# TSultanov/cfd-demo

Hardware: AMD Instinct MI355X
Metric: cell-updates/s (Poisson iter) + ms/timestep, 4096² grid, 1/2/4/8 GPU (higher is better)
Workload: dtype f32

## Files before the change

### cfd-demo_amd/cfdamd/__init__.py

```python
from __future__ import annotations

import ctypes as C
import enum
from dataclasses import dataclass
from typing import List, Optional, Tuple

import numpy as np

from . import _lib
from ._lib import (CFD_ENONFINITE, CfdError, CfdGrid, CfdParams, CfdResiduals, CfdState, check,
                   load)

__all__ = [
    "VelocityScheme", "InletProfile", "PressureSolver", "BoundaryKind", "Cylinder", "Grid",
    "SimulationParams", "Residuals", "SimSnapshot", "Model", "SimulationControlHandle",
    "CfdError", "default_grid", "cavity_grid", "rccl_unique_id", "device_count", "load", "LocalHub",
    "VisualizationMode", "CFD_ENONFINITE", "ScriptScheme", "ScriptPhase", "ScriptReport",
]


class VelocityScheme(enum.IntEnum):
    FirstOrder = 0
    SecondOrder = 1

# ... 464 lines not shown
        mm = np.empty(2, np.float32)
        check("cfd_derive_field", load().cfd_derive_field(self._hh(), int(mode), _fp(out), _fp(mm)))
        return out, (float(mm[0]), float(mm[1]))

    def launches_per_solve(self) -> int:
        tmax = self.kernel_config["temporal"]
        iters = self.params.jacobi_iters
        hg = self.halo_depth if self.n_ranks > 1 else 0
        T, lo, hi, ex = C.c_int(), C.c_int(), C.c_int(), C.c_int()
        it = n = 0
        while it < iters:
            check("cfd_plan_block", load().cfd_plan_block(
                self.j0, self.nyl, self.grid.ny, hg, it, tmax, iters, C.byref(T), C.byref(lo),
                C.byref(hi), C.byref(ex)))
            it += T.value
            n += 1
        return n

    @property
    def jacobi_kernel(self) -> dict:
        kind, name = C.c_int(), C.create_string_buffer(96)
        check("cfd_get_jacobi_kernel",
              load().cfd_get_jacobi_kernel(self._hh(), C.byref(kind), name, 96))
        return {"kind": kind.value, "name": name.value.decode()}

    def jacobi_geometry(self, persist: bool = True) -> dict:
        v = [C.c_int32() for _ in range(4)]
        check("cfd_get_jacobi_geometry",
              load().cfd_get_jacobi_geometry(self._hh(), int(bool(persist)), *(C.byref(x) for x in v)))
        return dict(lds_pad=v[0].value, wgs_per_cu=v[1].value, wave_cols=v[2].value,
                    segments=v[3].value)

    @property
    def persist_steals(self) -> int:
        n = C.c_uint64()
        check("cfd_get_persist_steals", load().cfd_get_persist_steals(self._hh(), C.byref(n)))
        return int(n.value)

    @property
    def persist_sums(self) -> int:
        n = C.c_uint64()
        check("cfd_get_persist_sums", load().cfd_get_persist_sums(self._hh(), C.byref(n)))
        return int(n.value)

    @property
    def sums_launches(self) -> int:
        n = C.c_uint64()
        check("cfd_get_sums_launches", load().cfd_get_sums_launches(self._hh(), C.byref(n)))
        return int(n.value)

    @property
    def sums_bounds(self) -> dict:
        s, a, b = C.c_uint32(), C.c_uint32(), C.c_uint32()
        check("cfd_get_sums_bounds",
              load().cfd_get_sums_bounds(self._hh(), C.byref(s), C.byref(a), C.byref(b)))
        return {"state": int(s.value), "m0": int(a.value), "rm": int(b.value)}

    @property
    def comm_calls(self) -> int:
        n = C.c_uint64()
        check("cfd_get_comm_calls", load().cfd_get_comm_calls(self._hh(), C.byref(n)))
        return int(n.value)

    @property
    def recoveries(self) -> int:
        n = C.c_uint64()
# ... 192 lines not shown
```

### cfd-demo_amd/cfdamd/_lib.py

```python
from __future__ import annotations

import ctypes as C
import os

PKG_DIR = os.path.dirname(os.path.abspath(__file__))
ROOT = os.path.dirname(PKG_DIR)
LIB_PATH = os.environ.get("CFD_LIB") or os.path.join(ROOT, "lib", "libcfd_amd.so")

EXPORTS = [
    "cfd_default_params", "cfd_default_grid", "cfd_create", "cfd_rccl_unique_id",
    "cfd_create_sharded", "cfd_local_hub_create", "cfd_local_hub_destroy",
    "cfd_create_sharded_local", "cfd_device_count", "cfd_get_comm_size", "cfd_get_slab", "cfd_update", "cfd_update_n", "cfd_piso_step",
    "cfd_pressure_solve", "cfd_run_phase", "cfd_set_params", "cfd_get_snapshot",
    "cfd_get_residuals", "cfd_get_state", "cfd_set_state", "cfd_get_masks", "cfd_synchronize",
    "cfd_profile_sweeps", "cfd_timing_begin", "cfd_timing_end", "cfd_timing_phases",
    "cfd_timing_phase_ms", "cfd_timing_exchange_ms", "cfd_get_halo_depth",
    "cfd_get_kernel_config", "cfd_get_jacobi_kernel", "cfd_get_persist_blocks", "cfd_get_persist_steals", "cfd_get_persist_sums", "cfd_get_sums_launches", "cfd_get_sums_bounds", "cfd_get_recoveries", "cfd_get_comm_calls", "cfd_get_resident_solves", "cfd_get_resident_geometry", "cfd_get_jacobi_geometry", "cfd_plan_slab", "cfd_plan_sweep", "cfd_plan_halo", "cfd_plan_block", "cfd_plan_overlap",
    "cfd_render", "cfd_derive_field", "cfd_last_error", "cfd_abi_version", "cfd_destroy",
    "cfd_get_config", "cfd_run_start", "cfd_run_stop", "cfd_run_pause", "cfd_run_resume",
    "cfd_run_set_params", "cfd_run_request_snapshot", "cfd_run_last_snapshot",
    "cfd_run_new_residuals", "cfd_run_status", "cfd_run_steps",
    "cfd_polygon_new", "cfd_polygon_new_rect", "cfd_polygon_new_regular", "cfd_polygon_add_hole",
    "cfd_polygon_contains_point", "cfd_polygon_intersects_aabb",
    "cfd_polygon_edges_intersect_aabb", "cfd_polygon_bounding_box",
    "cfd_polygon_bounding_square", "cfd_polygon_edges", "cfd_polygon_destroy",
    "cfd_geom_do_intersect", "cfd_geom_segment_intersection", "cfd_geom_intersect_quad_edge",
    "cfd_tesselate", "cfd_quadtree_size", "cfd_quadtree_nodes", "cfd_quadtree_destroy",
    "cfd_mesh_from_quadtree", "cfd_mesh_sizes", "cfd_mesh_cells", "cfd_mesh_neighbors",
    "cfd_mesh_intersections", "cfd_mesh_full_bounding_box", "cfd_mesh_build_ms",
    "cfd_mesh_destroy",
    "cfd_tracers_enable", "cfd_tracers_disable", "cfd_tracers_count", "cfd_tracers_get",
    "cfd_tracers_set", "cfd_tracers_advance", "cfd_tracers_inject", "cfd_tracers_density",
    "cfd_run_set_tracers", "cfd_run_last_tracers",
    "cfd_script_piso_step", "cfd_script_phase",
    "cfd_script_begin", "cfd_script_get_state", "cfd_script_set_state", "cfd_script_update",
    "cfd_script_update_n",
    "cfd_script_set_options", "cfd_script_get_options", "cfd_get_p_residual_f64",
]


class CfdGrid(C.Structure):
    _fields_ = [("nx", C.c_uint64), ("ny", C.c_uint64), ("lx", C.c_float), ("ly", C.c_float),
                ("has_cylinder", C.c_int32), ("cylinder_x", C.c_float),
                ("cylinder_y", C.c_float), ("cylinder_radius", C.c_float)]


class CfdParams(C.Structure):
    _fields_ = [("dt", C.c_float), ("viscosity", C.c_float),
                ("target_inlet_velocity", C.c_float), ("velocity_scheme", C.c_int32),
                ("inlet_profile", C.c_int32), ("pressure_solver", C.c_int32),
# ... 94 lines not shown
        "cfd_update_n": (i32, [vp, i32]),
        "cfd_piso_step": (i32, [vp, f32]),
        "cfd_pressure_solve": (i32, [vp, FP]),
        "cfd_run_phase": (i32, [vp, i32, f32]),
        "cfd_set_params": (i32, [vp, C.POINTER(CfdParams)]),
        "cfd_get_snapshot": (i32, [vp, FP, FP, FP, FP]),
        "cfd_get_residuals": (i32, [vp, C.POINTER(CfdResiduals)]),
        "cfd_get_state": (i32, [vp, C.POINTER(CfdState)]),
        "cfd_set_state": (i32, [vp, C.POINTER(CfdState)]),
        "cfd_get_masks": (i32, [vp, C.POINTER(C.c_uint8), C.POINTER(C.c_uint8)]),
        "cfd_synchronize": (i32, [vp]),
        "cfd_profile_sweeps": (i32, [vp, i32, C.POINTER(C.c_double)]),
        "cfd_timing_begin": (i32, [vp]),
        "cfd_timing_end": (i32, [vp, C.POINTER(C.c_double), C.POINTER(C.c_uint64),
                                 C.POINTER(C.c_double), C.POINTER(C.c_uint64)]),
        "cfd_timing_phases": (i32, [vp, i32]),
        "cfd_timing_phase_ms": (i32, [vp, C.POINTER(C.c_double), C.POINTER(C.c_double)]),
        "cfd_timing_exchange_ms": (i32, [vp, C.POINTER(C.c_double), C.POINTER(C.c_uint64)]),
        "cfd_get_halo_depth": (i32, [vp]),
        "cfd_get_kernel_config": (i32, [vp, C.POINTER(i32), C.POINTER(i32)]),
        "cfd_get_jacobi_kernel": (i32, [vp, C.POINTER(i32), C.c_char_p, C.c_size_t]),
        "cfd_get_persist_blocks": (i32, [vp, C.POINTER(i32)]),
        "cfd_get_persist_steals": (i32, [vp, C.POINTER(C.c_uint64)]),
        "cfd_get_persist_sums": (i32, [vp, C.POINTER(C.c_uint64)]),
        "cfd_get_sums_launches": (i32, [vp, C.POINTER(C.c_uint64)]),
        "cfd_get_sums_bounds": (i32, [vp, C.POINTER(C.c_uint32), C.POINTER(C.c_uint32),
                                      C.POINTER(C.c_uint32)]),
        "cfd_get_recoveries": (i32, [vp, C.POINTER(C.c_uint64)]),
        "cfd_get_comm_calls": (i32, [vp, C.POINTER(C.c_uint64)]),
        "cfd_get_resident_solves": (i32, [vp, C.POINTER(C.c_uint64)]),
        "cfd_get_resident_geometry": (i32, [vp] + [C.POINTER(i32)] * 4),
        "cfd_get_jacobi_geometry": (i32, [vp, i32, C.POINTER(i32), C.POINTER(i32), C.POINTER(i32),
                                          C.POINTER(i32)]),
        "cfd_plan_slab": (i32, [C.c_uint64, i32, i32, C.POINTER(C.c_uint64),
                                C.POINTER(C.c_uint64)]),
        "cfd_plan_sweep": (i32, [i32, i32, i32, i32, i32, i32, C.POINTER(i32), C.POINTER(i32),
                                 C.POINTER(i32)]),
        "cfd_plan_halo": (i32, [i32, i32, i32, i32, i32, C.POINTER(i32)]),
        "cfd_plan_overlap": (i32, [i32, i32, i32, i32, i32, i32, C.POINTER(i32)]),
        "cfd_plan_block": (i32, [i32, i32, i32, i32, i32, i32, i32, C.POINTER(i32),
                                 C.POINTER(i32), C.POINTER(i32), C.POINTER(i32)]),
        "cfd_render": (i32, [vp, i32, C.POINTER(C.c_uint8), FP]),
        "cfd_derive_field": (i32, [vp, i32, FP, FP]),
        "cfd_last_error": (C.c_char_p, []),
        "cfd_abi_version": (i32, []),
        "cfd_destroy": (None, [vp]),
        "cfd_get_config": (i32, [vp, C.POINTER(CfdGrid), C.POINTER(CfdParams)]),
        "cfd_run_start": (i32, [vp, C.POINTER(vp)]),
        "cfd_run_stop": (i32, [vp]),
        "cfd_run_pause": (i32, [vp]),
        "cfd_run_resume": (i32, [vp]),
        "cfd_run_set_params": (i32, [vp, C.POINTER(CfdParams)]),
        "cfd_run_request_snapshot": (i32, [vp]),
        "cfd_run_last_snapshot": (i32, [vp, FP, FP, FP, FP, C.POINTER(i32), C.POINTER(i32)]),
        "cfd_run_new_residuals": (i32, [vp, C.POINTER(CfdResiduals), i32, C.POINTER(i32)]),
        "cfd_run_status": (i32, [vp, C.c_char_p, C.c_size_t]),
        "cfd_run_steps": (C.c_uint64, [vp]),
        "cfd_polygon_new": (i32, [C.POINTER(CfdPoint), C.c_size_t, C.POINTER(C.c_uint64),
                                  C.c_size_t, C.POINTER(vp), C.POINTER(i32)]),
        "cfd_polygon_new_rect": (i32, [C.c_double] * 4 + [C.POINTER(vp)]),
        "cfd_polygon_new_regular": (i32, [CfdPoint, C.c_double, C.c_size_t, C.c_double,
                                          C.POINTER(vp)]),
        "cfd_polygon_add_hole": (i32, [vp, vp, C.POINTER(i32)]),
        "cfd_polygon_contains_point": (i32, [vp, CfdPoint, C.POINTER(i32)]),
        "cfd_polygon_intersects_aabb": (i32, [vp, C.POINTER(CfdAabb), C.POINTER(i32)]),
        "cfd_polygon_edges_intersect_aabb": (i32, [vp, C.POINTER(CfdAabb), C.POINTER(i32)]),
# ... 59 lines not shown
```

### cfd-demo_amd/csrc/cfd_internal.h

```cpp
#pragma once
#include <hip/hip_runtime.h>
#include <stdint.h>

#include <type_traits>

#include "../../include/cfd.h"

namespace cfd {

template <class Fn>
auto with_fastdiv(int fastdiv, Fn &&f) {
    if (fastdiv == 1) return f(std::integral_constant<int, 1>{});
    if (fastdiv == 2) return f(std::integral_constant<int, 2>{});
    return f(std::integral_constant<int, 0>{});
}

constexpr int kGhostUV = 2;
constexpr float kSumsPLim = 0x1p122f, kSumsRLim = 0x1p112f;
constexpr int kMaxSweeps = 4096;
constexpr int kMaxPasses = 64;

constexpr int kResSlots = 32;
constexpr int kResStride = 16;
constexpr int kPersistFlagStride = 16;
// ... 68 lines not shown
    size_t u_alloc, v_alloc;
    float *u_alloc_base, *v_alloc_base, *u_old_base, *v_old_base, *u_star_base, *v_star_base;
    Ctl *ctl;
    uint32_t *host_nonfinite;
    uint32_t *host_progress;
    uint32_t *persist;
    int32_t sums_track;
};

inline bool aligned16(const void *p) { return ((uintptr_t)p & 15u) == 0; }

void launch_step_begin(const Geom &g, const Fields &f, int copy, hipStream_t s);
void launch_copy_star(const Geom &g, const Fields &f, int pass, hipStream_t s);
void launch_copy_star_div(const Geom &g, const Fields &f, int pass, float dt_override,
                          hipStream_t s);
void launch_u_predictor(const Geom &g, const Fields &f, float dt_override, hipStream_t s);
void launch_v_predictor(const Geom &g, const Fields &f, float dt_override, hipStream_t s);
void launch_predict(const Geom &g, const Fields &f, float dt_override, bool vec, hipStream_t s);
bool predict_march_ok(const Geom &g, const Fields &f);
int predict_march_workgroups(const Geom &g);
void launch_predict_march(const Geom &g, const Fields &f, float dt_override, hipStream_t s,
                          bool set_inlet = false, int row_lo = 0, int row_hi = -1, int mode = 0,
                          bool star = false);
void launch_divergence(const Geom &g, const Fields &f, int pass, float dt_override,
                       hipStream_t s);
void launch_jacobi_sweep(const Geom &g, const Fields &f, int pass, int it, int row_lo,
                         int row_hi, int res, hipStream_t s);
void launch_jacobi_block(const Geom &g, const Fields &f, int pass, int it, int par, int T,
                         int out_lo, int out_hi, int res, hipStream_t s);
bool launch_jacobi_persist(const Geom &g, const Fields &f, int pass, int par0, int nblk,
                           int out_lo, int out_hi, uint32_t epoch, int res_it, hipStream_t s);
void lds_geometry8(const Geom &g, int out_lo, int out_hi, bool persist, int *pad, int *occ, int *nwc,
                   int *nseg);
void launch_tb1(const Geom &g, const Fields &f, int T, int pass, int it, int par, int out_lo,
                int out_hi, uint32_t *res_slots, hipStream_t s);
void launch_pipe(const Geom &g, const Fields &f, int T, int pass, int it, int par, int out_lo,
                 int out_hi, uint32_t *res_slots, hipStream_t s);
bool launch_lds_persist8(const Geom &g, const Fields &f, int pass, int par0, int nblk, int out_lo,
                         int out_hi, uint32_t epoch, uint32_t *rs, hipStream_t s);
void launch_lds(const Geom &g, const Fields &f, int T, int pass, int it, int par, int out_lo,
                int out_hi, uint32_t *res_slots, hipStream_t s, int mode = 0, int lag = 0);
void launch_jacobi_spec(const Geom &g, const Fields &f, int pass, int it, int par, int T,
                        int out_lo, int out_hi, hipStream_t s, int lag = 0);
void launch_spec_check(const Geom &g, const Fields &f, int pass, int it, int T, int par,
                       hipStream_t s);
bool launch_jacobi_resident(const Geom &g, const Fields &f, int pass, int iters, int fin,
                            int check_break, hipStream_t s);
bool jacobi_resident_geometry(const Geom &g, int *br, int *bc, int *tiles, int *wgs);
void launch_spec_align(const Geom &g, const Fields &f, int pass, int n, hipStream_t s);
void launch_jacobi_redo(const Geom &g, const Fields &f, int pass, int out_lo, int out_hi,
                        hipStream_t s, int last_it = 0, int last_par = 0, int last_T = 0);
void launch_fold_slots(uint32_t *dst, uint32_t *slots, int n, hipStream_t s);
void launch_vis_field(const Geom &g, const Fields &f, int mode, float *out, uint32_t *slots,
                      hipStream_t s);
void launch_vis_color(const Geom &g, const Fields &f, int mode, const float *field, uint32_t *px,
                      const uint32_t *keys, int has_cyl, float cx, float cy, float radius,
                      hipStream_t s);
void launch_verify_division(float c, float r, unsigned long long *dev_counts, hipStream_t s);
void launch_finalize_solve(const Geom &g, const Fields &f, int pass, int iters, int check_break,
                           int flips, hipStream_t s, int exact_flips = 0);

struct SorConst {
    double dx2, dy2, denom;
    double r_dx2, r_dy2, r_denom;
    int32_t fast;
};
// ... 108 lines not shown
```

### cfd-demo_amd/csrc/cfd_jacobi_lds.h

```cpp
#pragma once
#include <cmath>
#include <type_traits>

#include "cfd_device.h"

#ifndef CFD_LDS_PD
#define CFD_LDS_PD 3
#endif
#ifndef CFD_LDS_SPLIT
#define CFD_LDS_SPLIT 1
#endif
#ifndef CFD_LDS_PRIO
#define CFD_LDS_PRIO 1
#endif
#ifndef CFD_LDS_ST_AUX
#define CFD_LDS_ST_AUX 16
#endif
#ifndef CFD_LDS_SPEC_WPE
#define CFD_LDS_SPEC_WPE 5
#endif
#ifndef CFD_PERSIST_WPE
#define CFD_PERSIST_WPE 3
#endif
#ifndef CFD_LDS_STAMP
#define CFD_LDS_STAMP 0
#endif

namespace cfd {

constexpr int kLdsWaves = 4;

#if CFD_LDS_STAMP
namespace {
constexpr int kStampWaves = 1 << 15;
__device__ unsigned long long g_lds_stamp[kStampWaves * 4];
template <bool RES>
struct StampOnExit {
    unsigned long long rt0, t0;
    unsigned long long bid;
    __device__ explicit StampOnExit(int b)
        : rt0(__builtin_amdgcn_s_memrealtime()), t0(__builtin_amdgcn_s_memtime()),
          bid((unsigned long long)b) {}
    __device__ ~StampOnExit() {
        if (RES) return;
        const unsigned long long rt1 = __builtin_amdgcn_s_memrealtime();
        const unsigned long long t1 = __builtin_amdgcn_s_memtime();
        const unsigned hw = __builtin_amdgcn_s_getreg(4 | (31 << 11));
        const unsigned xcc = __builtin_amdgcn_s_getreg(20 | (31 << 11));
        const int idx = (int)blockIdx.x * kLdsWaves + ((int)threadIdx.x >> 6);
        if ((threadIdx.x & 63) == 0 && idx < kStampWaves) {
            g_lds_stamp[idx * 4 + 0] = rt0;
            g_lds_stamp[idx * 4 + 1] = rt1;
            g_lds_stamp[idx * 4 + 2] = (bid << 40) | ((t1 - t0) & 0xFFFFFFFFFFull);
            g_lds_stamp[idx * 4 + 3] = ((unsigned long long)xcc << 32) | hw;
        }
    }
};
}
extern "C" int cfd_diag_lds_stamps(unsigned long long *host, int nwaves) {
    if (nwaves > kStampWaves) nwaves = kStampWaves;
    return hipMemcpyFromSymbol(host, HIP_SYMBOL(g_lds_stamp), (size_t)nwaves * 32, 0,
                               hipMemcpyDeviceToHost) == hipSuccess ? nwaves : -1;
}
#endif

constexpr int lds_outl(int T) { return 64 - 2 * ((T + 1) / 2); }

struct LdsTiles {
    int pad, nwc, nseg, wlo, whi;
};
LdsTiles lds_tiles(const Geom &g, int T, int out_lo, int out_hi, int mode, int bpc, bool one_round);
int lds_pad_bytes(const Geom &g, int mode);
bool lds_sums_grid(const Geom &g);

void launch_lds_t567(const Geom &g, const Fields &f, int T, int pass, int par, int it, int out_lo,
                     int out_hi, uint32_t *rs, int mode, hipStream_t s, int lag);
void launch_lds_t8(const Geom &g, const Fields &f, int pass, int par, int it, int out_lo, int out_hi,
                   uint32_t *rs, int mode, hipStream_t s, int lag);
int persist_blocks_per_cu8(const Geom &g, int pad);

namespace {

typedef unsigned int u32x2 __attribute__((ext_vector_type(2)));
constexpr int lds_gcd(int a, int b) { return b == 0 ? a : lds_gcd(b, a % b); }
constexpr int lds_off(int s, int T, int G) { return s <= 0 ? 0 : ((s - 1) * G) / T; }
constexpr int lds_nw(int G) { return G > 1 ? 4 : 3; }
constexpr int ring_depth(int T, int PD, int G) {
    const int nw = lds_nw(G);
    const int q = nw / lds_gcd(nw, PD) * PD;
    const int need = T + lds_off(T, T, G) + 1;
    return ((need + q - 1) / q) * q;
}

template <int T, int FAST, int MODE, int SUMS = 0>
struct LdsMarch {
    static constexpr bool RES = MODE == 1 || MODE == 5, SPEC = MODE == 2, REDO = MODE == 3;
    static constexpr bool PERSIST = MODE == 4 || MODE == 5;
    static constexpr bool TRACK_IN = PERSIST && !SUMS;
    static constexpr bool TRACK_OUT = PERSIST;
    static_assert(!SUMS || FAST == 1, "SUMS: reciprocal multiply");
    static constexpr int PLD_AUX = PERSIST ? 16 : 0;
    static constexpr int PST_AUX = PERSIST ? 16 : CFD_LDS_ST_AUX;
    static constexpr int G = CFD_LDS_SPLIT;
    static constexpr int NW = lds_nw(G);
    static constexpr int PD = CFD_LDS_PD;
    static constexpr int OFFT = lds_off(T, T, G);
    static constexpr int D = ring_depth(T, PD, G);
    static constexpr int U = D;
    static constexpr int WARM = 2 * T + OFFT;
    static constexpr int H = (T + 1) / 2;
    static constexpr int OUTL = lds_outl(T);
    static constexpr int off(int s) { return lds_off(s, T, G); }
    static constexpr int start(int s) { return 2 * s + off(s); }
    static_assert(D % PD == 0 && D % NW == 0 && D >= T + OFFT + 1, "ring geometry");
    static_assert(G >= 1 && G <= T, "stage groups");

    f2 W[T][NW];
    f2 PQ[PD];
    f2 RQ[PD];
    f2 *ring;
    int lane;
    int k_first, S, lo_clamp, hi_clamp, nch, g_first, g_last, g_top, g_zero, row_bytes;
    int wbase;
    int ch, vo_ld, vo_st, abase, dir;
    bool e0, e1;
    float dx_sq, r_dx_sq, dy_sq, r_dy_sq, denom, r_denom;
    __amdgpu_buffer_rsrc_t rs_p, rs_r, rs_d;
    float m;
    float omax, imax, rmax;
    float mm[SPEC ? T : 1];
    int r0v, r1v;
    int nst;
    int nyl_;

    LdsMarch() = default;

    __device__ __forceinline__ int act(int vrow) const { return abase + dir * vrow; }

    template <int AUX = 0>
    __device__ __forceinline__ f2 ld(__amdgpu_buffer_rsrc_t rs, int vrow) const {
        vrow = vrow < k_first + S ? vrow : k_first + S - 1;
        int row = act(vrow);
        row = row < lo_clamp ? lo_clamp : (row > hi_clamp ? hi_clamp : row);
        const u32x2 v = __builtin_amdgcn_raw_buffer_load_b64(rs, vo_ld, (row - wbase) * row_bytes, AUX);
        return (f2){__uint_as_float(v.x), __uint_as_float(v.y)};
    }
    __device__ __forceinline__ void st(const f2 &x, int row) const {
        const u32x2 v = {__float_as_uint(x.x), __float_as_uint(x.y)};
// ... 79 lines not shown
                    }
                }
            }
            if (REDO && s == nst) {
                if (r >= r0v && r < r1v) {
                    const int ra = act(r);
                    st(n, ra);
                    if ((E & kRow) && r == g_first) st(n, g_zero);
                    if ((E & kRow) && r == g_last) st(n, g_top);
                }
            } else if (s < T) {
                if ((E & kRow) && r == g_top) n = W[s][(V_ - 1 + kW) % NW];
                W[s][V_ % NW] = n;
                if ((E & kRow) && r == g_first) W[s][(V_ - 1 + kW) % NW] = n;
            } else {
                const int ra = act(r);
                if (RES && ra >= 0 && ra < nyl_) {
                    const f2 d = n - C;
                    if (!(E & kCol)) {
                        m = fmaxf(fmaxf(m, fabsf(d.x)), fabsf(d.y));
                    } else {
                        if (e0) m = fmaxf(m, fabsf(d.x));
                        if (e1) m = fmaxf(m, fabsf(d.y));
                    }
                }
                st(n, ra);
                if ((E & kRow) && r == g_first) st(n, g_zero);
                if ((E & kRow) && r == g_last) st(n, g_top);
                if constexpr (TRACK_OUT) omax = fmaxf(fmaxf(omax, fabsf(n.x)), fabsf(n.y));
            }
        }
    }

    template <int V_, int E>
    __device__ __forceinline__ void warmup() {
        if constexpr (V_ < WARM) {
            slot<V_, 0, E>(V_);
            warmup<V_ + 1, E>();
        }
    }

    template <int J, int GUARD, int E>
    __device__ __forceinline__ void group(int base) {
        if constexpr (J < U) {
            slot<WARM + J, GUARD, E>(base + J);
            group<J + 1, GUARD, E>(base);
        }
    }

    __device__ __forceinline__ void set_prio(int done) const {
        if (!CFD_LDS_PRIO) return;
        const int rows = S - WARM, d4 = 4 * done;
        if (d4 >= 3 * rows)
            __builtin_amdgcn_s_setprio(0);
        else if (d4 >= 2 * rows)
            __builtin_amdgcn_s_setprio(1);
        else if (d4 >= rows)
            __builtin_amdgcn_s_setprio(2);
        else
            __builtin_amdgcn_s_setprio(3);
    }

    template <int E>
    __device__ __forceinline__ void run() {
        set_prio(0);
        warmup<0, E>();
        int base = WARM;
        const int full_end = WARM + ((S - WARM) / U) * U;
        for (; base < full_end; base += U) {
            set_prio(base - WARM);
            group<0, 1, E>(base);
        }
        set_prio(base - WARM);
        if (base < S) group<0, 2, E>(base);
    }
};

template <int T, int FAST, int MODE, int SUMS = 0>
__device__ __forceinline__ void lds_block(const Geom &g, float *__restrict__ pa,
                                          float *__restrict__ pb, const float *__restrict__ rhs,
                                          Ctl *ctl, uint32_t *res_slots, int par, int out_lo,
                                          int out_hi, int nwc, int nseg, int wlo, int whi, f2 *lds,
                                          int nst, int bid, float *trk = nullptr) {
    using M = LdsMarch<T, FAST, MODE, SUMS>;
    constexpr bool RES = M::RES;
    M w;
    w.nst = nst;
    const int wave = __builtin_amdgcn_readfirstlane((int)threadIdx.x >> 6);
    const int lane = (int)threadIdx.x & 63;
    if (M::PERSIST && trk && lane == 0) trk[3 * wave] = trk[3 * wave + 1] = trk[3 * wave + 2] = 0.0f;
    const int wc = bid % nwc;
    const int seg = (bid / nwc) * kLdsWaves + wave;
    const int nrows = out_hi - out_lo;
    if (seg >= nseg) return;
    const long total = nseg == 1 ? 16 : wlo + whi + 16L * (nseg - 2);
    auto cum = [&](int i) -> long { return i <= 0 ? 0 : (i >= nseg ? total : wlo + 16L * (i - 1)); };
    const int r0 = out_lo + (int)(cum(seg) * nrows / total);
    const int r1 = out_lo + (int)(cum(seg + 1) * nrows / total);
    if (r0 >= r1) return;
    const int nx = g.nx;
    w.ring = lds + wave * M::D * 64;
    w.lane = lane;
    w.nch = nx / 2;
    w.nyl_ = g.nyl;
    w.lo_clamp = -g.hg;
    w.hi_clamp = g.nyl + g.hg - 1;
    w.ch = wc * M::OUTL - M::H + lane;
    const bool in_dom = w.ch >= 0 && w.ch < w.nch;
    const bool out_lane = in_dom && lane >= M::H && lane < 64 - M::H;
    const int col = 2 * w.ch;
    w.row_bytes = nx * 4;
    constexpr int kFar = 0x7FFF0000;
    w.vo_ld = in_dom ? col * 4 : kFar;
    w.vo_st = out_lane ? col * 4 : kFar;
    const int si = (ctl->cur + par) & 1;
    float *src_alloc = si ? pb : pa;
    float *dst_alloc = si ? pa : pb;
// ... 121 lines not shown
            if (stop_s) return;
            if (spec_lag_first(g, ctl, res_slots - (size_t)lag * kResSlots * kResStride, it - lag, lag,
                               par - 1) < lag)
                return;
        } else if (ctl->spec_stop) {
            return;
        }
    }
    if constexpr (M::REDO) {
        if (lag > 0 && !ctl->spec_stop) {
            const int j = spec_lag_first(g, ctl, res_slots, it, lag, par, false);
            nst = j + 1 < lag ? j + 1 : 0;
        } else {
            nst = ctl->spec_redo;
            par = ctl->spec_launch;
        }
        if (nst <= 0) return;
    }
    if constexpr (FAST == 1 && MODE <= 1) {
        if (sums_c > 0.0f && ctl->sums_state == 2u) {
            const float bound = __uint_as_float(ctl->sums_m0) * g.r_dx_sq + sums_c * __uint_as_float(ctl->sums_rm);
            if (bound < 0x1p123f) {
                if (blockIdx.x == 0 && threadIdx.x == 0) atomicAdd(&ctl->sums_launches, 1u);
                lds_block<T, FAST, MODE, 2>(g, pa, pb, rhs, ctl, res_slots, par, out_lo, out_hi, nwc, nseg,
                                            wlo, whi, lds, nst, xcd_block(g));
                return;
            }
        }
    }
    lds_block<T, FAST, MODE>(g, pa, pb, rhs, ctl, res_slots, par, out_lo, out_hi, nwc, nseg, wlo,
                             whi, lds, nst, xcd_block(g));
}

template <int T, int FAST, int MODE>
int lds_blocks_per_cu(int pad) {
    static int cache[2] = {0, 0};
    int &nb = cache[pad > 0 ? 1 : 0];
    if (nb == 0) {
        int n = 0;
        if (hipOccupancyMaxActiveBlocksPerMultiprocessor(
                &n, reinterpret_cast<const void *>(&k_jacobi_lds<T, FAST, MODE>), kLdsWaves * 64, pad) !=
                hipSuccess ||
            n < 1)
            n = 1;
        nb = n;
    }
    return nb;
}

template <int T, int MODE>
void launch_lds_t(const Geom &g, const Fields &f, int pass, int par, int it, int out_lo, int out_hi,
                  uint32_t *rs, hipStream_t s, int lag = 0) {
    const int bpc = with_fastdiv(g.fastdiv, [&](auto F) {
        return lds_blocks_per_cu<T, F(), MODE>(lds_pad_bytes(g, MODE));
    });
    const LdsTiles t = lds_tiles(g, T, out_lo, out_hi, MODE, bpc, false);
    const dim3 grid(t.nwc * cdiv(t.nseg, kLdsWaves)), block(kLdsWaves * 64);
    float *pa = f.pp[0] - (long)g.hg * g.nx, *pb = f.pp[1] - (long)g.hg * g.nx;
    const float sums_c =
        MODE <= 1 && g.j0 == 0 && g.nyl == g.ny && lds_sums_grid(g) ? 0.1875f * kMaxSweeps : 0.0f;
    with_fastdiv(g.fastdiv, [&](auto F) {
        hipLaunchKernelGGL((k_jacobi_lds<T, F(), MODE>), grid, block, t.pad, s, g, pa, pb, f.rhs, f.ctl,
                           rs, pass, par, out_lo, out_hi, t.nwc, t.nseg, t.wlo, t.whi, it, lag, sums_c);
    });
}

template <int T>
void launch_lds_T(const Geom &g, const Fields &f, int pass, int par, int it, int out_lo, int out_hi,
                  uint32_t *rs, int mode, hipStream_t s, int lag = 0) {
    if (mode == 2) {
        launch_lds_t<T, 2>(g, f, pass, par, it, out_lo, out_hi, rs, s, lag);
        return;
    }
    if constexpr (T == 8) {
        if (mode == 3) {
            launch_lds_t<8, 3>(g, f, pass, par, it, out_lo, out_hi, rs, s, lag);
            return;
        }
    }
    if (rs)
        launch_lds_t<T, 1>(g, f, pass, par, it, out_lo, out_hi, rs, s);
    else
        launch_lds_t<T, 0>(g, f, pass, par, it, out_lo, out_hi, rs, s);
}

}
}
```

### cfd-demo_amd/csrc/cfd_jacobi_lds8.hip

```cpp
#include "cfd_jacobi_lds.h"

namespace cfd {

void launch_lds_t8(const Geom &g, const Fields &f, int pass, int par, int it, int out_lo, int out_hi,
                   uint32_t *rs, int mode, hipStream_t s, int lag) {
    launch_lds_T<8>(g, f, pass, par, it, out_lo, out_hi, rs, mode, s, lag);
}

void lds_geometry8(const Geom &g, int out_lo, int out_hi, bool persist, int *pad, int *occ, int *nwc,
                   int *nseg) {
    const int pd = lds_pad_bytes(g, 0);
    const int o = persist ? persist_blocks_per_cu8(g, pd)
                          : with_fastdiv(g.fastdiv, [&](auto F) { return lds_blocks_per_cu<8, F(), 0>(pd); });
    const LdsTiles t = lds_tiles(g, 8, out_lo, out_hi, 0, o, persist);
    if (pad) *pad = t.pad;
    if (occ) *occ = o;
    if (nwc) *nwc = t.nwc;
    if (nseg) *nseg = t.nseg;
}

}
```

### cfd-demo_amd/csrc/cfd_model_abi.hip

```cpp
#include <cstddef>
#include <cstdio>
#include <cstring>

#include "cfd_model.h"

using namespace cfd;

namespace {
thread_local std::string g_last_error;
}

int cfd::fail(int code, const std::string &msg) {
    g_last_error = msg;
    return code;
}

extern "C" {

const char *cfd_last_error(void) { return g_last_error.c_str(); }
void cfdrt_set_error(const char *msg) { g_last_error = msg ? msg : ""; }
int cfdrt_check_params(const cfd_model *m, const cfd_params *p) {
    if (!m) return fail(CFD_EINVAL, "null model");
    int rc = validate(&m->grid, p);
    if (rc) return rc;
// ... 545 lines not shown
            snprintf(buf, sizeof buf, "k_jacobi_resident<%d>", m->g.res_div);
        else if (spec)
            snprintf(buf, sizeof buf, "k_jacobi_lds<%d, %d, 2>", T, m->g.fastdiv);
        else if (k == 0)
            snprintf(buf, sizeof buf, "k_jacobi<%d, %d>", kJacRowsPerWave, m->g.fastdiv);
        else if (k == 1)
            snprintf(buf, sizeof buf, "k_jacobi_tb<%d, %d>", T, m->g.fastdiv);
        else if (k == 5)
            snprintf(buf, sizeof buf, "k_jacobi_lds<%d, %d, 0>", T, m->g.fastdiv);
        else
            snprintf(buf, sizeof buf, "k_jacobi_pipe<%d, %d>", T, m->g.fastdiv);
        snprintf(name, name_len, "%s", buf);
    }
    return 0;
}

int cfd_get_jacobi_geometry(const cfd_model *m, int persist, int *lds_pad, int *wgs_per_cu,
                            int *wave_cols, int *segments) {
    if (!m) return fail(CFD_EINVAL, "null model");
    if (hipSetDevice(m->device) != hipSuccess) return fail(CFD_EHIP, "hipSetDevice");
    int T, lo, hi, exch;
    plan_block((int)m->j0, m->g.nyl, m->g.ny, m->sharded() ? m->g.hg : 0, 0, 8,
               std::max(8, m->params.jacobi_iters), &T, &lo, &hi, &exch);
    if (!m->sharded()) lo = 1 - (int)m->j0, hi = (int)m->g.ny - 1 - (int)m->j0;
    int pad = 0, occ = 0, nwc = 0, nseg = 0;
    lds_geometry8(m->g, lo, hi, persist != 0, &pad, &occ, &nwc, &nseg);
    if (lds_pad) *lds_pad = pad;
    if (wgs_per_cu) *wgs_per_cu = occ;
    if (wave_cols) *wave_cols = nwc;
    if (segments) *segments = nseg;
    return 0;
}

int cfd_get_persist_steals(cfd_model *m, uint64_t *steals) {
    if (!m || !steals) return fail(CFD_EINVAL, "null argument");
    int rc = m->sync();
    if (rc) return rc;
    uint32_t v = 0;
    HIP_TRY(hipMemcpy(&v, m->f.persist + 2, 4, hipMemcpyDeviceToHost));
    *steals = v;
    return 0;
}

int cfd_get_persist_sums(cfd_model *m, uint64_t *blocks) {
    if (!m || !blocks) return fail(CFD_EINVAL, "null argument");
    int rc = m->sync();
    if (rc) return rc;
    uint32_t v = 0;
    HIP_TRY(hipMemcpy(&v, m->f.persist + 3, 4, hipMemcpyDeviceToHost));
    *blocks = v;
    return 0;
}

int cfd_get_sums_launches(cfd_model *m, uint64_t *launches) {
    if (!m || !launches) return fail(CFD_EINVAL, "null argument");
    Ctl c;
    int rc = m->read_ctl(&c);
    if (rc) return rc;
    *launches = c.sums_launches;
    return 0;
}

int cfd_get_sums_bounds(cfd_model *m, uint32_t *state, uint32_t *m0_bits, uint32_t *rm_bits) {
    if (!m || !state || !m0_bits || !rm_bits) return fail(CFD_EINVAL, "null argument");
    Ctl c;
    int rc = m->read_ctl(&c);
// ... 85 lines not shown
```

### include/cfd.h

```cpp
#ifndef CFD_H
#define CFD_H

#include <stddef.h>
#include <stdint.h>

#ifdef __cplusplus
extern "C" {
#endif

#define CFD_ABI_VERSION 1

typedef enum {
    CFD_OK = 0,
    CFD_EINVAL = -1,
    CFD_EHIP = -2,
    CFD_ERCCL = -3,
    CFD_ESTATE = -4,
    CFD_ENONFINITE = -5,
    CFD_ETIMEOUT = -6,
} cfd_status;

typedef struct cfd_model cfd_model;

typedef struct {
// ... 73 lines not shown
int cfd_run_phase(cfd_model *m, int phase, float dt_sub);

int cfd_set_params(cfd_model *m, const cfd_params *params);
int cfd_get_snapshot(cfd_model *m, float *u, float *v, float *p, float *dt_out);
int cfd_get_residuals(cfd_model *m, cfd_residuals *out);
int cfd_get_state(cfd_model *m, cfd_state *st);
int cfd_set_state(cfd_model *m, const cfd_state *st);
int cfd_get_masks(cfd_model *m, uint8_t *mask_u, uint8_t *mask_v);

int cfd_synchronize(cfd_model *m);
int cfd_profile_sweeps(cfd_model *m, int n_sweeps, double *avg_ms_out);

int cfd_timing_begin(cfd_model *m);
int cfd_timing_end(cfd_model *m, double *solve_ms, uint64_t *sweeps, double *step_ms,
                   uint64_t *steps);
int cfd_timing_phases(cfd_model *m, int on);
int cfd_timing_phase_ms(const cfd_model *m, double *predict_ms, double *finish_ms);
int cfd_timing_exchange_ms(const cfd_model *m, double *exchange_ms, uint64_t *exchanges);
int cfd_get_halo_depth(const cfd_model *m);
int cfd_get_kernel_config(const cfd_model *m, int *fastdiv, int *temporal);
int cfd_get_jacobi_kernel(const cfd_model *m, int *kind, char *name, size_t name_len);

int cfd_get_persist_blocks(const cfd_model *m, int *blocks);
int cfd_get_persist_steals(cfd_model *m, uint64_t *steals);
int cfd_get_persist_sums(cfd_model *m, uint64_t *blocks);
int cfd_get_sums_launches(cfd_model *m, uint64_t *launches);
int cfd_get_sums_bounds(cfd_model *m, uint32_t *state, uint32_t *m0_bits, uint32_t *rm_bits);
int cfd_get_comm_calls(const cfd_model *m, uint64_t *n);
int cfd_get_recoveries(const cfd_model *m, uint64_t *n);
int cfd_get_resident_solves(const cfd_model *m, uint64_t *solves);
int cfd_get_resident_geometry(const cfd_model *m, int *br, int *bc, int *tiles, int *wgs);
int cfd_get_jacobi_geometry(const cfd_model *m, int persist, int *lds_pad, int *wgs_per_cu,
                            int *wave_cols, int *segments);

int cfd_plan_slab(uint64_t ny, int n_ranks, int rank, uint64_t *j0, uint64_t *j1);
int cfd_plan_sweep(int j0, int nyl, int ny, int halo_depth, int it, int iters, int *lo, int *hi,
                   int *exchange);
int cfd_plan_halo(int kind, int nyl, int depth, int rank, int n_ranks, int *out6);
int cfd_plan_overlap(int nyl, int halo_depth, int rank, int n_ranks, int lo, int hi, int *out6);
int cfd_plan_block(int j0, int nyl, int ny, int halo_depth, int it, int t_max, int iters, int *T,
                   int *out_lo, int *out_hi, int *exchange);

typedef enum { CFD_VIS_PRESSURE = 0, CFD_VIS_VELOCITY = 1, CFD_VIS_VORTICITY = 2 } cfd_vis_mode;

int cfd_render(cfd_model *m, int mode, uint8_t *rgba, float *min_max_out);
int cfd_derive_field(cfd_model *m, int mode, float *out, float *min_max_out);

int cfd_tracers_enable(cfd_model *m, uint64_t capacity, int inject_interval);
int cfd_tracers_disable(cfd_model *m);
int cfd_tracers_count(cfd_model *m, uint64_t *n);
int cfd_tracers_get(cfd_model *m, double *x, double *y, double *initial_y, uint64_t max,
                    uint64_t *n_out);
int cfd_tracers_set(cfd_model *m, const double *x, const double *y, const double *initial_y,
                    uint64_t n);
int cfd_tracers_advance(cfd_model *m, double dt);
int cfd_tracers_inject(cfd_model *m);
int cfd_tracers_density(cfd_model *m, uint32_t *counts_nx_ny);

enum { CFD_SCRIPT_FIRST = 0, CFD_SCRIPT_SECOND = 1, CFD_SCRIPT_QUICK = 2 };
typedef struct {
    int32_t scheme;
    int32_t inlet_profile;
    double  inlet_velocity;
    double  dt_sub;
} cfd_script_step;
int cfd_script_piso_step(cfd_model *m, const cfd_script_step *s);
// ... 107 lines not shown
```

Before: 2916 billion.

## Process two rows per ring slot in the T=8 LDS Jacobi march kernel

```diff
diff --git a/cfd-demo_amd/cfdamd/__init__.py b/cfd-demo_amd/cfdamd/__init__.py
--- a/cfd-demo_amd/cfdamd/__init__.py
+++ b/cfd-demo_amd/cfdamd/__init__.py
@@ -520,6 +520,13 @@
                     segments=v[3].value)
 
     @property
+    def jacobi_rows_per_slot(self) -> int:
+        n = C.c_int32()
+        check("cfd_get_jacobi_rows_per_slot",
+              load().cfd_get_jacobi_rows_per_slot(self._hh(), C.byref(n)))
+        return int(n.value)
+
+    @property
     def persist_steals(self) -> int:
         n = C.c_uint64()
         check("cfd_get_persist_steals", load().cfd_get_persist_steals(self._hh(), C.byref(n)))
diff --git a/cfd-demo_amd/cfdamd/_lib.py b/cfd-demo_amd/cfdamd/_lib.py
--- a/cfd-demo_amd/cfdamd/_lib.py
+++ b/cfd-demo_amd/cfdamd/_lib.py
@@ -15,7 +15,7 @@
     "cfd_get_residuals", "cfd_get_state", "cfd_set_state", "cfd_get_masks", "cfd_synchronize",
     "cfd_profile_sweeps", "cfd_timing_begin", "cfd_timing_end", "cfd_timing_phases",
     "cfd_timing_phase_ms", "cfd_timing_exchange_ms", "cfd_get_halo_depth",
-    "cfd_get_kernel_config", "cfd_get_jacobi_kernel", "cfd_get_persist_blocks", "cfd_get_persist_steals", "cfd_get_persist_sums", "cfd_get_sums_launches", "cfd_get_sums_bounds", "cfd_get_recoveries", "cfd_get_comm_calls", "cfd_get_resident_solves", "cfd_get_resident_geometry", "cfd_get_jacobi_geometry", "cfd_plan_slab", "cfd_plan_sweep", "cfd_plan_halo", "cfd_plan_block", "cfd_plan_overlap",
+    "cfd_get_kernel_config", "cfd_get_jacobi_kernel", "cfd_get_persist_blocks", "cfd_get_persist_steals", "cfd_get_persist_sums", "cfd_get_sums_launches", "cfd_get_sums_bounds", "cfd_get_recoveries", "cfd_get_comm_calls", "cfd_get_resident_solves", "cfd_get_resident_geometry", "cfd_get_jacobi_geometry", "cfd_get_jacobi_rows_per_slot", "cfd_plan_slab", "cfd_plan_sweep", "cfd_plan_halo", "cfd_plan_block", "cfd_plan_overlap",
     "cfd_render", "cfd_derive_field", "cfd_last_error", "cfd_abi_version", "cfd_destroy",
     "cfd_get_config", "cfd_run_start", "cfd_run_stop", "cfd_run_pause", "cfd_run_resume",
     "cfd_run_set_params", "cfd_run_request_snapshot", "cfd_run_last_snapshot",
@@ -176,6 +176,7 @@
         "cfd_get_resident_geometry": (i32, [vp] + [C.POINTER(i32)] * 4),
         "cfd_get_jacobi_geometry": (i32, [vp, i32, C.POINTER(i32), C.POINTER(i32), C.POINTER(i32),
                                           C.POINTER(i32)]),
+        "cfd_get_jacobi_rows_per_slot": (i32, [vp, C.POINTER(i32)]),
         "cfd_plan_slab": (i32, [C.c_uint64, i32, i32, C.POINTER(C.c_uint64),
                                 C.POINTER(C.c_uint64)]),
         "cfd_plan_sweep": (i32, [i32, i32, i32, i32, i32, i32, C.POINTER(i32), C.POINTER(i32),
diff --git a/cfd-demo_amd/csrc/cfd_internal.h b/cfd-demo_amd/csrc/cfd_internal.h
--- a/cfd-demo_amd/csrc/cfd_internal.h
+++ b/cfd-demo_amd/csrc/cfd_internal.h
@@ -124,6 +124,7 @@
                            int out_lo, int out_hi, uint32_t epoch, int res_it, hipStream_t s);
 void lds_geometry8(const Geom &g, int out_lo, int out_hi, bool persist, int *pad, int *occ, int *nwc,
                    int *nseg);
+int lds_rows_per_slot(const Geom &g, int T, int mode);
 void launch_tb1(const Geom &g, const Fields &f, int T, int pass, int it, int par, int out_lo,
                 int out_hi, uint32_t *res_slots, hipStream_t s);
 void launch_pipe(const Geom &g, const Fields &f, int T, int pass, int it, int par, int out_lo,
diff --git a/cfd-demo_amd/csrc/cfd_jacobi_lds.h b/cfd-demo_amd/csrc/cfd_jacobi_lds.h
--- a/cfd-demo_amd/csrc/cfd_jacobi_lds.h
+++ b/cfd-demo_amd/csrc/cfd_jacobi_lds.h
@@ -9,6 +9,9 @@
 #endif
 #ifndef CFD_LDS_SPLIT
 #define CFD_LDS_SPLIT 1
+#endif
+#ifndef CFD_LDS_ROWS
+#define CFD_LDS_ROWS 2
 #endif
 #ifndef CFD_LDS_PRIO
 #define CFD_LDS_PRIO 1
@@ -72,6 +75,7 @@
 LdsTiles lds_tiles(const Geom &g, int T, int out_lo, int out_hi, int mode, int bpc, bool one_round);
 int lds_pad_bytes(const Geom &g, int mode);
 bool lds_sums_grid(const Geom &g);
+int lds_rows_per_slot(const Geom &g, int T, int mode);
 
 void launch_lds_t567(const Geom &g, const Fields &f, int T, int pass, int par, int it, int out_lo,
                      int out_hi, uint32_t *rs, int mode, hipStream_t s, int lag);
@@ -91,8 +95,13 @@
     const int need = T + lds_off(T, T, G) + 1;
     return ((need + q - 1) / q) * q;
 }
-
-template <int T, int FAST, int MODE, int SUMS = 0>
+constexpr int ring_depth2(int T, int PD) {
+    const int q = 4 / lds_gcd(4, PD) * PD;
+    return ((T + 2 + q - 1) / q) * q;
+}
+constexpr int lds_rps(int T, int MODE) { return CFD_LDS_ROWS == 2 && T == 8 && MODE <= 1 ? 2 : 1; }
+
+template <int T, int FAST, int MODE, int SUMS = 0, int RPS = 1>
 struct LdsMarch {
     static constexpr bool RES = MODE == 1 || MODE == 5, SPEC = MODE == 2, REDO = MODE == 3;
     static constexpr bool PERSIST = MODE == 4 || MODE == 5;
@@ -102,10 +111,10 @@
     static constexpr int PLD_AUX = PERSIST ? 16 : 0;
     static constexpr int PST_AUX = PERSIST ? 16 : CFD_LDS_ST_AUX;
     static constexpr int G = CFD_LDS_SPLIT;
-    static constexpr int NW = lds_nw(G);
+    static constexpr int NW = RPS == 2 ? 4 : lds_nw(G);
     static constexpr int PD = CFD_LDS_PD;
     static constexpr int OFFT = lds_off(T, T, G);
-    static constexpr int D = ring_depth(T, PD, G);
+    static constexpr int D = RPS == 2 ? ring_depth2(T, PD) : ring_depth(T, PD, G);
     static constexpr int U = D;
     static constexpr int WARM = 2 * T + OFFT;
     static constexpr int H = (T + 1) / 2;
@@ -114,6 +123,7 @@
     static constexpr int start(int s) { return 2 * s + off(s); }
     static_assert(D % PD == 0 && D % NW == 0 && D >= T + OFFT + 1, "ring geometry");
     static_assert(G >= 1 && G <= T, "stage groups");
+    static_assert(RPS == 1 || (RPS == 2 && G == 1 && MODE <= 1 && D >= T + 2), "two rows per slot");
 
     f2 W[T][NW];
     f2 PQ[PD];
@@ -259,19 +269,120 @@
         }
     }
 
+    __device__ __forceinline__ void update2(const f2 &B, const f2 &C, const f2 &T0, const f2 &T1,
+                                            const f2 &Rh0, const f2 &Rh1, f2 &n0, f2 &n1) const {
+        const float hx0 = C.y + from_left(C.y);
+        const float hx1 = T0.y + from_left(T0.y);
+        const float hy0 = C.x + from_right(C.x);
+        const float hy1 = T0.x + from_right(T0.x);
+        const f2 h0 = {hx0, hy0}, h1 = {hx1, hy1};
+        const f2 v0 = T0 + B, v1 = T1 + C;
+        const float omega = 0.75f;
+        const float om1 = 1.0f - omega;
+        if constexpr (SUMS == 2) {
+            const f2 s0 = h0 + v0, s1 = h1 + v1;
+            const f2 d0 = __builtin_elementwise_fma(s0, (f2){r_dx_sq, r_dx_sq}, -Rh0);
+            const f2 d1 = __builtin_elementwise_fma(s1, (f2){r_dx_sq, r_dx_sq}, -Rh1);
+            const f2 pu0 = d0 * r_denom, pu1 = d1 * r_denom;
+            const f2 a0 = 0.75f * pu0, a1 = 0.75f * pu1;
+            n0 = a0 + 0.25f * C;
+            n1 = a1 + 0.25f * T0;
+        } else {
+            const f2 hz0 = fdiv2<FAST>(h0, dx_sq, r_dx_sq), hz1 = fdiv2<FAST>(h1, dx_sq, r_dx_sq);
+            const f2 vt0 = fdiv2<FAST>(v0, dy_sq, r_dy_sq), vt1 = fdiv2<FAST>(v1, dy_sq, r_dy_sq);
+            const f2 s0 = hz0 + vt0, s1 = hz1 + vt1;
+            const f2 e0_ = s0 - Rh0, e1_ = s1 - Rh1;
+            const f2 pu0 = fdiv2<FAST>(e0_, denom, r_denom), pu1 = fdiv2<FAST>(e1_, denom, r_denom);
+            n0 = omega * pu0 + om1 * C;
+            n1 = omega * pu1 + om1 * T0;
+        }
+    }
+
+    __device__ __forceinline__ void col_patch(f2 &o) const {
+        if (ch == 0) o.x = o.y;
+        if (ch == nch - 1) o.y = 0.0f;
+    }
+
+    template <int E>
+    __device__ __forceinline__ void finish_row(const f2 &n, const f2 &C, int r) {
+        const int ra = act(r);
+        if (RES && ra >= 0 && ra < nyl_) {
+            const f2 d = n - C;
+            if (!(E & kCol)) {
+                m = fmaxf(fmaxf(m, fabsf(d.x)), fabsf(d.y));
+            } else {
+                if (e0) m = fmaxf(m, fabsf(d.x));
+                if (e1) m = fmaxf(m, fabsf(d.y));
+            }
+        }
+        st(n, ra);
+        if ((E & kRow) && r == g_first) st(n, g_zero);
+        if ((E & kRow) && r == g_last) st(n, g_top);
+    }
+
+    template <int V_, int GUARD, int E>
+    __device__ __forceinline__ void slot2(int v) {
+        static_assert(V_ % 2 == 0, "slots start at even rows");
+        if (GUARD == 2 && v >= S) return;
+        const bool two = GUARD != 2 || v + 1 < S;
+        const int k = k_first + v;
+        W[0][V_ % 4] = PQ[V_ % PD];
+        W[0][(V_ + 1) % 4] = PQ[(V_ + 1) % PD];
+        PQ[V_ % PD] = ld(rs_p, k + PD);
+        PQ[(V_ + 1) % PD] = ld(rs_p, k + 1 + PD);
+        ring[(V_ % D) * 64 + lane] = RQ[V_ % PD];
+        ring[((V_ + 1) % D) * 64 + lane] = RQ[(V_ + 1) % PD];
+        RQ[V_ % PD] = ld(rs_r, k + PD);
+        RQ[(V_ + 1) % PD] = ld(rs_r, k + 1 + PD);
+#pragma unroll
+        for (int s = 1; s <= T; ++s) {
+            if (GUARD == 0 && V_ < start(s)) continue;
+            const int r = k - s;
+            const f2 rh0 = ring[((V_ - s + 8 * D) % D) * 64 + lane];
+            const f2 rh1 = ring[((V_ + 1 - s + 8 * D) % D) * 64 + lane];
+            const f2 &B = W[s - 1][(V_ + 2) % 4];
+            const f2 &C = W[s - 1][(V_ + 3) % 4];
+            const f2 &T0 = W[s - 1][V_ % 4];
+            const f2 &T1 = W[s - 1][(V_ + 1) % 4];
+            f2 n0, n1;
+            update2(B, C, T0, T1, rh0, rh1, n0, n1);
+            if (E & kCol) {
+                col_patch(n0);
+                col_patch(n1);
+            }
+            if (s < T) {
+                if ((E & kRow) && r == g_top) n0 = W[s][(V_ + 3) % 4];
+                W[s][V_ % 4] = n0;
+                if ((E & kRow) && r == g_first) W[s][(V_ + 3) % 4] = n0;
+                if ((E & kRow) && r + 1 == g_top) n1 = n0;
+                W[s][(V_ + 1) % 4] = n1;
+                if ((E & kRow) && two && r + 1 == g_first) W[s][V_ % 4] = n1;
+            } else {
+                finish_row<E>(n0, C, r);
+                if (two) finish_row<E>(n1, T0, r + 1);
+            }
+        }
+    }
+
     template <int V_, int E>
     __device__ __forceinline__ void warmup() {
         if constexpr (V_ < WARM) {
-            slot<V_, 0, E>(V_);
-            warmup<V_ + 1, E>();
+            if constexpr (RPS == 2)
+                slot2<V_, 0, E>(V_);
+            else
+                slot<V_, 0, E>(V_);
+            warmup<V_ + RPS, E>();
         }
     }
 
     template <int J, int GUARD, int E>
     __device__ __forceinline__ void group(int base) {
         if constexpr (J < U) {
-            slot<WARM + J, GUARD, E>(base + J);
-            group<J + 1, GUARD, E>(base);
+            if constexpr (RPS == 2)
+                slot2<WARM + J, GUARD, E>(base + J);
+            else
+                slot<WARM + J, GUARD, E>(base + J);
+            group<J + RPS, GUARD, E>(base);
         }
     }
 
@@ -303,13 +414,13 @@
     }
 };
 
-template <int T, int FAST, int MODE, int SUMS = 0>
+template <int T, int FAST, int MODE, int SUMS = 0, int RPS = 1>
 __device__ __forceinline__ void lds_block(const Geom &g, float *__restrict__ pa,
                                           float *__restrict__ pb, const float *__restrict__ rhs,
                                           Ctl *ctl, uint32_t *res_slots, int par, int out_lo,
                                           int out_hi, int nwc, int nseg, int wlo, int whi, f2 *lds,
                                           int nst, int bid, float *trk = nullptr) {
-    using M = LdsMarch<T, FAST, MODE, SUMS>;
+    using M = LdsMarch<T, FAST, MODE, SUMS, RPS>;
     constexpr bool RES = M::RES;
     M w;
     w.nst = nst;
@@ -497,6 +608,32 @@
                              whi, lds, nst, xcd_block(g));
 }
 
+#if CFD_LDS_ROWS == 2
+template <int FAST, int MODE>
+__global__ __launch_bounds__(kLdsWaves * 64, 1) void k_jacobi_lds_rows2(
+    Geom g, float *__restrict__ pa, float *__restrict__ pb, const float *__restrict__ rhs,
+    Ctl *ctl, uint32_t *res_slots, int pass, int par, int out_lo, int out_hi, int nwc, int nseg,
+    int wlo, int whi, int it, int lag, float sums_c) {
+    static_assert(MODE <= 1, "plain and RES launches");
+    using M = LdsMarch<8, FAST, MODE, 0, 2>;
+    __shared__ f2 lds[kLdsWaves * M::D * 64];
+    if (pass_off(ctl, pass)) return;
+    if constexpr (FAST == 1) {
+        if (sums_c > 0.0f && ctl->sums_state == 2u) {
+            const float bound = __uint_as_float(ctl->sums_m0) * g.r_dx_sq + sums_c * __uint_as_float(ctl->sums_rm);
+            if (bound < 0x1p123f) {
+                if (blockIdx.x == 0 && threadIdx.x == 0) atomicAdd(&ctl->sums_launches, 1u);
+                lds_block<8, FAST, MODE, 2, 2>(g, pa, pb, rhs, ctl, res_slots, par, out_lo, out_hi, nwc, nseg,
+                                               wlo, whi, lds, 0, xcd_block(g));
+                return;
+            }
+        }
+    }
+    lds_block<8, FAST, MODE, 0, 2>(g, pa, pb, rhs, ctl, res_slots, par, out_lo, out_hi, nwc, nseg, wlo, whi,
+                                   lds, 0, xcd_block(g));
+}
+#endif
+
 template <int T, int FAST, int MODE>
 int lds_blocks_per_cu(int pad) {
     static int cache[2] = {0, 0};
@@ -512,18 +649,56 @@
     }
     return nb;
 }
+#if CFD_LDS_ROWS == 2
+template <int FAST, int MODE>
+int lds_blocks_per_cu_rows2(int pad) {
+    static int cache[2] = {0, 0};
+    int &nb = cache[pad > 0 ? 1 : 0];
+    if (nb == 0) {
+        int n = 0;
+        if (hipOccupancyMaxActiveBlocksPerMultiprocessor(
+                &n, reinterpret_cast<const void *>(&k_jacobi_lds_rows2<FAST, MODE>), kLdsWaves * 64, pad) !=
+                hipSuccess ||
+            n < 1)
+            n = 1;
+        nb = n;
+    }
+    return nb;
+}
+#endif
+template <int T, int MODE>
+int lds_launch_blocks_per_cu(const Geom &g) {
+    const int pad = lds_pad_bytes(g, MODE);
+#if CFD_LDS_ROWS == 2
+    if constexpr (lds_rps(T, MODE) == 2) {
+        if (lds_rows_per_slot(g, T, MODE) == 2)
+            return with_fastdiv(g.fastdiv, [&](auto F) { return lds_blocks_per_cu_rows2<F(), MODE>(pad); });
+    }
+#endif
+    return with_fastdiv(g.fastdiv, [&](auto F) { return lds_blocks_per_cu<T, F(), MODE>(pad); });
+}
 
 template <int T, int MODE>
 void launch_lds_t(const Geom &g, const Fields &f, int pass, int par, int it, int out_lo, int out_hi,
                   uint32_t *rs, hipStream_t s, int lag = 0) {
-    const int bpc = with_fastdiv(g.fastdiv, [&](auto F) {
-        return lds_blocks_per_cu<T, F(), MODE>(lds_pad_bytes(g, MODE));
-    });
+    const int bpc = lds_launch_blocks_per_cu<T, MODE>(g);
     const LdsTiles t = lds_tiles(g, T, out_lo, out_hi, MODE, bpc, false);
     const dim3 grid(t.nwc * cdiv(t.nseg, kLdsWaves)), block(kLdsWaves * 64);
     float *pa = f.pp[0] - (long)g.hg * g.nx, *pb = f.pp[1] - (long)g.hg * g.nx;
     const float sums_c =
         MODE <= 1 && g.j0 == 0 && g.nyl == g.ny && lds_sums_grid(g) ? 0.1875f * kMaxSweeps : 0.0f;
+#if CFD_LDS_ROWS == 2
+    if constexpr (lds_rps(T, MODE) == 2) {
+        if (lds_rows_per_slot(g, T, MODE) == 2) {
+            with_fastdiv(g.fastdiv, [&](auto F) {
+                hipLaunchKernelGGL((k_jacobi_lds_rows2<F(), MODE>), grid, block, t.pad, s, g, pa, pb, f.rhs,
+                                   f.ctl, rs, pass, par, out_lo, out_hi, t.nwc, t.nseg, t.wlo, t.whi, it, lag,
+                                   sums_c);
+            });
+            return;
+        }
+    }
+#endif
     with_fastdiv(g.fastdiv, [&](auto F) {
         hipLaunchKernelGGL((k_jacobi_lds<T, F(), MODE>), grid, block, t.pad, s, g, pa, pb, f.rhs, f.ctl,
                            rs, pass, par, out_lo, out_hi, t.nwc, t.nseg, t.wlo, t.whi, it, lag, sums_c);
diff --git a/cfd-demo_amd/csrc/cfd_jacobi_lds8.hip b/cfd-demo_amd/csrc/cfd_jacobi_lds8.hip
--- a/cfd-demo_amd/csrc/cfd_jacobi_lds8.hip
+++ b/cfd-demo_amd/csrc/cfd_jacobi_lds8.hip
@@ -7,11 +7,16 @@
     launch_lds_T<8>(g, f, pass, par, it, out_lo, out_hi, rs, mode, s, lag);
 }
 
+int lds_rows_per_slot(const Geom &g, int T, int mode) {
+    const char *ue = getenv("CFD_JACOBI_ROWS");
+    if (ue && atoi(ue) == 1) return 1;
+    return lds_rps(T, mode) == 2 && g.j0 == 0 && g.nyl == g.ny ? 2 : 1;
+}
+
 void lds_geometry8(const Geom &g, int out_lo, int out_hi, bool persist, int *pad, int *occ, int *nwc,
                    int *nseg) {
     const int pd = lds_pad_bytes(g, 0);
-    const int o = persist ? persist_blocks_per_cu8(g, pd)
-                          : with_fastdiv(g.fastdiv, [&](auto F) { return lds_blocks_per_cu<8, F(), 0>(pd); });
+    const int o = persist ? persist_blocks_per_cu8(g, pd) : lds_launch_blocks_per_cu<8, 0>(g);
     const LdsTiles t = lds_tiles(g, 8, out_lo, out_hi, 0, o, persist);
     if (pad) *pad = t.pad;
     if (occ) *occ = o;
diff --git a/cfd-demo_amd/csrc/cfd_model_abi.hip b/cfd-demo_amd/csrc/cfd_model_abi.hip
--- a/cfd-demo_amd/csrc/cfd_model_abi.hip
+++ b/cfd-demo_amd/csrc/cfd_model_abi.hip
@@ -601,6 +601,12 @@
     return 0;
 }
 
+int cfd_get_jacobi_rows_per_slot(const cfd_model *m, int *rows) {
+    if (!m || !rows) return fail(CFD_EINVAL, "null argument");
+    *rows = lds_rows_per_slot(m->g, 8, 0);
+    return 0;
+}
+
 int cfd_get_persist_steals(cfd_model *m, uint64_t *steals) {
     if (!m || !steals) return fail(CFD_EINVAL, "null argument");
     int rc = m->sync();
diff --git a/include/cfd.h b/include/cfd.h
--- a/include/cfd.h
+++ b/include/cfd.h
@@ -129,6 +129,7 @@
 int cfd_get_resident_geometry(const cfd_model *m, int *br, int *bc, int *tiles, int *wgs);
 int cfd_get_jacobi_geometry(const cfd_model *m, int persist, int *lds_pad, int *wgs_per_cu,
                             int *wave_cols, int *segments);
+int cfd_get_jacobi_rows_per_slot(const cfd_model *m, int *rows);
 
 int cfd_plan_slab(uint64_t ny, int n_ranks, int rank, uint64_t *j0, uint64_t *j1);
 int cfd_plan_sweep(int j0, int nyl, int ny, int halo_depth, int it, int iters, int *lo, int *hi,
```

Measured after the change: 2941 billion (median of 6 runs). No clear change (+0.8%).
